# zwang86/FlexFlow

Measured on AMD Instinct MI355X. Metric: samples/sec under auto-searched strategy at 1/2/4/8 MI355X; speedup vs DP, higher is better.
Workload: dtype bf16; 1 GPU; model=bert-large, global_batch=32, seq_len=512, parallelism=single, search=data_parallel, optimizer=adam, params=366426938, hidden=1024, layers=24, heads=16, vocab=30522, vocab_padded=30528

## Files before the change

csrc/kernels/norm.hip:

```cpp
#include "common.h"
#include "ops.h"

namespace ffk {

template <typename T, int NCH>
__global__ void __launch_bounds__(256) ln_fwd_kernel(const T* __restrict__ x, const T* __restrict__ res,
                                                     T* __restrict__ sum_out, const T* __restrict__ gamma,
                                                     const T* __restrict__ beta, T* __restrict__ y,
                                                     float* __restrict__ mean_out, float* __restrict__ rstd_out,
                                                     int rows, int cols, float eps) {
  constexpr int V = 16 / sizeof(T);
  const int lane = threadIdx.x & 63;
  const int wave = (blockIdx.x * blockDim.x + threadIdx.x) >> 6;
  const int nwaves = (gridDim.x * blockDim.x) >> 6;
  for (int row = wave; row < rows; row += nwaves) {
    const int64_t base = (int64_t)row * cols;
    float v[NCH][V];
    float s = 0.f;
#pragma unroll
    for (int c = 0; c < NCH; ++c) {
      const int col = (c * 64 + lane) * V;
      if (col < cols) {
        load16(x + base + col, v[c]);
        if (res) {
          float r[V];
          load16(res + base + col, r);
#pragma unroll
          for (int j = 0; j < V; ++j) v[c][j] += r[j];
          if (sum_out) store16(sum_out + base + col, v[c]);
        }
#pragma unroll
        for (int j = 0; j < V; ++j) s += v[c][j];
      } else {
#pragma unroll
        for (int j = 0; j < V; ++j) v[c][j] = 0.f;
      }
    }
    const float mean = wave_sum(s) / cols;
    float q = 0.f;
#pragma unroll
    for (int c = 0; c < NCH; ++c) {
      const int col = (c * 64 + lane) * V;
      if (col < cols) {
#pragma unroll
        for (int j = 0; j < V; ++j) { const float d = v[c][j] - mean; q += d * d; }
      }
    }
    const float rstd = rsqrtf(wave_sum(q) / cols + eps);
    if (lane == 0) { mean_out[row] = mean; rstd_out[row] = rstd; }
#pragma unroll
    for (int c = 0; c < NCH; ++c) {
      const int col = (c * 64 + lane) * V;
      if (col < cols) {
        float g[V], bb[V], o[V];
        if (gamma) load16(gamma + col, g); else for (int j = 0; j < V; ++j) g[j] = 1.f;
        if (beta) load16(beta + col, bb); else for (int j = 0; j < V; ++j) bb[j] = 0.f;
#pragma unroll
        for (int j = 0; j < V; ++j) o[j] = (v[c][j] - mean) * rstd * g[j] + bb[j];
        store16(y + base + col, o);
      }
    }
  }
}

template <typename T>
__global__ void ln_fwd_generic(const T* __restrict__ x, const T* __restrict__ res, T* __restrict__ sum_out,
                               const T* __restrict__ gamma, const T* __restrict__ beta, T* __restrict__ y,
                               float* __restrict__ mean_out, float* __restrict__ rstd_out, int rows, int cols,
                               float eps) {
  const int lane = threadIdx.x & 63;
  const int wave = (blockIdx.x * blockDim.x + threadIdx.x) >> 6;
  const int nwaves = (gridDim.x * blockDim.x) >> 6;
  for (int row = wave; row < rows; row += nwaves) {
    const int64_t base = (int64_t)row * cols;
    float s = 0.f;
    for (int c = lane; c < cols; c += 64) {
      float v = Cvt<T>::to_f(x[base + c]);
      if (res) { v += Cvt<T>::to_f(res[base + c]); if (sum_out) sum_out[base + c] = Cvt<T>::from_f(v); }
      s += v;
    }
    const float mean = wave_sum(s) / cols;
    float q = 0.f;
    for (int c = lane; c < cols; c += 64) {
      float v = Cvt<T>::to_f(x[base + c]) + (res ? Cvt<T>::to_f(res[base + c]) : 0.f);
      q += (v - mean) * (v - mean);
    }
    const float rstd = rsqrtf(wave_sum(q) / cols + eps);
    if (lane == 0) { mean_out[row] = mean; rstd_out[row] = rstd; }
    for (int c = lane; c < cols; c += 64) {
      float v = Cvt<T>::to_f(x[base + c]) + (res ? Cvt<T>::to_f(res[base + c]) : 0.f);
      float g = gamma ? Cvt<T>::to_f(gamma[c]) : 1.f;
      float b = beta ? Cvt<T>::to_f(beta[c]) : 0.f;
      y[base + c] = Cvt<T>::from_f((v - mean) * rstd * g + b);
    }
  }
}

template <typename T, int NCH, int NT = 256>
__global__ void __launch_bounds__(NT) ln_bwd_kernel(const T* __restrict__ dy, const T* __restrict__ x,
                                                     const T* __restrict__ gamma, const float* __restrict__ mean_in,
                                                     const float* __restrict__ rstd_in, T* __restrict__ dx,
                                                     const T* __restrict__ dres_in, float* __restrict__ pgam,
                                                     float* __restrict__ pbet, float* __restrict__ pdx, int rows,
                                                     int cols, int accumulate) {
  constexpr int V = 16 / sizeof(T);
  const int lane = threadIdx.x & 63;
  const int wave = (blockIdx.x * blockDim.x + threadIdx.x) >> 6;
  const int nwaves = (gridDim.x * blockDim.x) >> 6;
  float pg[NCH][V], pb[NCH][V], pd[NCH][V];
#pragma unroll
  for (int c = 0; c < NCH; ++c)
#pragma unroll
    for (int j = 0; j < V; ++j) { pg[c][j] = 0.f; pb[c][j] = 0.f; pd[c][j] = 0.f; }
  for (int row = wave; row < rows; row += nwaves) {
    const int64_t base = (int64_t)row * cols;
    const float mean = mean_in[row], rstd = rstd_in[row];
    float xh[NCH][V], gy[NCH][V];
    float s1 = 0.f, s2 = 0.f;
#pragma unroll
    for (int c = 0; c < NCH; ++c) {
      const int col = (c * 64 + lane) * V;
      if (col < cols) {
        float xv[V], dv[V], g[V];
        load16(x + base + col, xv);
        load16(dy + base + col, dv);
        if (gamma) load16(gamma + col, g); else for (int j = 0; j < V; ++j) g[j] = 1.f;
#pragma unroll
        for (int j = 0; j < V; ++j) {
          xh[c][j] = (xv[j] - mean) * rstd;
          pg[c][j] += dv[j] * xh[c][j];
          pb[c][j] += dv[j];
          gy[c][j] = dv[j] * g[j];
          s1 += gy[c][j];
          s2 += gy[c][j] * xh[c][j];
        }
      } else {
#pragma unroll
        for (int j = 0; j < V; ++j) { xh[c][j] = 0.f; gy[c][j] = 0.f; }
      }
    }
    s1 = wave_sum(s1) / cols;
    s2 = wave_sum(s2) / cols;
#pragma unroll
    for (int c = 0; c < NCH; ++c) {
      const int col = (c * 64 + lane) * V;
      if (col < cols) {
        float o[V];
#pragma unroll
        for (int j = 0; j < V; ++j) o[j] = rstd * (gy[c][j] - s1 - xh[c][j] * s2);
        if (dres_in) {
          float r[V];
          load16(dres_in + base + col, r);
#pragma unroll
          for (int j = 0; j < V; ++j) o[j] += r[j];
        }
        if (accumulate) {
          float r[V];
          load16(dx + base + col, r);
#pragma unroll
          for (int j = 0; j < V; ++j) o[j] += r[j];
        }
#pragma unroll
        for (int j = 0; j < V; ++j) pd[c][j] += o[j];
        store16(dx + base + col, o);
      }
    }
  }
  extern __shared__ float lds_red[];
  constexpr int NWB = NT / 64;
  const int w = threadIdx.x >> 6;
#pragma unroll
  for (int pass = 0; pass < 3; ++pass) {
    float* slab = pass == 2 ? pdx : (pass ? pbet : pgam);
    if (!slab) continue;
#pragma unroll
    for (int c = 0; c < NCH; ++c) {
      const int col = (c * 64 + lane) * V;
      if (col < cols)
#pragma unroll
        for (int j = 0; j < V; ++j) lds_red[w * cols + col + j] = pass == 2 ? pd[c][j] : (pass ? pb[c][j] : pg[c][j]);
    }
    __syncthreads();
    for (int k = threadIdx.x; k < cols; k += NT) {
      float t = 0.f;
#pragma unroll
      for (int q = 0; q < NWB; ++q) t += lds_red[q * cols + k];
      slab[(int64_t)blockIdx.x * cols + k] = t;
    }
    __syncthreads();
  }
}

template <typename T>
__global__ void ln_bwd_generic(const T* __restrict__ dy, const T* __restrict__ x, const T* __restrict__ gamma,
                               const float* __restrict__ mean_in, const float* __restrict__ rstd_in,
                               T* __restrict__ dx, const T* __restrict__ dres_in, float* __restrict__ dgamma,
                               float* __restrict__ dbeta, int rows, int cols, int accumulate) {
  const int lane = threadIdx.x & 63;
  const int wave = (blockIdx.x * blockDim.x + threadIdx.x) >> 6;
  const int nwaves = (gridDim.x * blockDim.x) >> 6;
  for (int row = wave; row < rows; row += nwaves) {
    const int64_t base = (int64_t)row * cols;
    const float mean = mean_in[row], rstd = rstd_in[row];
    float s1 = 0.f, s2 = 0.f;
    for (int c = lane; c < cols; c += 64) {
      const float xh = (Cvt<T>::to_f(x[base + c]) - mean) * rstd;
      const float d = Cvt<T>::to_f(dy[base + c]);
      const float g = (gamma ? Cvt<T>::to_f(gamma[c]) : 1.f) * d;
      s1 += g; s2 += g * xh;
      if (dgamma) atomicAdd(dgamma + c, d * xh);
      if (dbeta) atomicAdd(dbeta + c, d);
    }
    s1 = wave_sum(s1) / cols;
    s2 = wave_sum(s2) / cols;
    for (int c = lane; c < cols; c += 64) {
      const float xh = (Cvt<T>::to_f(x[base + c]) - mean) * rstd;
      const float g = (gamma ? Cvt<T>::to_f(gamma[c]) : 1.f) * Cvt<T>::to_f(dy[base + c]);
      float o = rstd * (g - s1 - xh * s2);
      if (dres_in) o += Cvt<T>::to_f(dres_in[base + c]);
      if (accumulate) o += Cvt<T>::to_f(dx[base + c]);
      dx[base + c] = Cvt<T>::from_f(o);
    }
  }
}

static bool a16(const void* p) { return ((uintptr_t)p & 15) == 0; }

static bool ln_bwd_wide_on() {
  static int v = -1;
  if (v < 0) {
    const char* e = getenv("FF_LN_BWD_WIDE");
    v = e ? atoi(e) : 0;
  }
  return v != 0;
}

void layernorm_fwd(int dt, const void* x, const void* res, void* sum_out, const void* gamma, const void* beta,
                   void* y, float* mean, float* rstd, int rows, int cols, float eps, hipStream_t st) {
  if (rows == 0) return;
  const int esz = dt == DT_BF16 ? 2 : 4;
  const int V = 16 / esz;
  const bool vec = (cols % V == 0) && a16(x) && a16(y) && (!res || a16(res)) && (!sum_out || a16(sum_out)) &&
                   (!gamma || a16(gamma)) && (!beta || a16(beta));
  const int nch = (cols + 64 * V - 1) / (64 * V);
  const int blocks = std::max(1, std::min((rows + 3) / 4, 4096));
#define LNF(T, N) hipLaunchKernelGGL((ln_fwd_kernel<T, N>), dim3(blocks), dim3(256), 0, st, (const T*)x, (const T*)res, \
                                     (T*)sum_out, (const T*)gamma, (const T*)beta, (T*)y, mean, rstd, rows, cols, eps)
  if (dt == DT_BF16) {
    using T = bf16_t;
    if (vec && nch <= 1) LNF(T, 1); else if (vec && nch <= 2) LNF(T, 2); else if (vec && nch <= 4) LNF(T, 4);
    else if (vec && nch <= 8) LNF(T, 8);
    else hipLaunchKernelGGL(ln_fwd_generic<T>, dim3(blocks), dim3(256), 0, st, (const T*)x, (const T*)res, (T*)sum_out,
                            (const T*)gamma, (const T*)beta, (T*)y, mean, rstd, rows, cols, eps);
  } else {
    using T = float;
    if (vec && nch <= 1) LNF(T, 1); else if (vec && nch <= 2) LNF(T, 2); else if (vec && nch <= 4) LNF(T, 4);
    else if (vec && nch <= 8) LNF(T, 8);
    else hipLaunchKernelGGL(ln_fwd_generic<T>, dim3(blocks), dim3(256), 0, st, (const T*)x, (const T*)res, (T*)sum_out,
                            (const T*)gamma, (const T*)beta, (T*)y, mean, rstd, rows, cols, eps);
  }
#undef LNF
}

int layernorm_bwd_waves(int rows) { return std::max(1, std::min((rows + 15) / 16, 1024)); }
static bool ln_bwd_wide(int cols) { return cols <= 1024 && ln_bwd_wide_on(); }
static int ln_bwd_blocks(int rows, int cols) {
  return ln_bwd_wide(cols) ? std::max(1, std::min((rows + 63) / 64, 256)) : layernorm_bwd_waves(rows);
}

void layernorm_bwd(int dt, const void* dy, const void* x, const void* gamma, const float* mean, const float* rstd,
                   void* dx, const void* dres_in, float* dgamma, float* dbeta, float* dsum, float* ws, int rows,
                   int cols, int accumulate, hipStream_t st, int stage) {
  if (rows == 0) return;
  const int esz = dt == DT_BF16 ? 2 : 4;
  const int V = 16 / esz;
  const bool vec = (cols % V == 0) && a16(x) && a16(dy) && a16(dx) && (!dres_in || a16(dres_in)) &&
                   (!gamma || a16(gamma));
  const int nch = (cols + 64 * V - 1) / (64 * V);
  const bool wide = ln_bwd_wide(cols);
  const int blocks = ln_bwd_blocks(rows, cols);
  const int nw = blocks;
  float* pg = dgamma ? ws : nullptr;
  float* pb = dbeta ? ws + (int64_t)nw * cols : nullptr;
  float* pd = dsum ? ws + 2 * (int64_t)nw * cols : nullptr;
  bool used_slab = false;
  const bool fused_ok = vec && nch <= 4;
  if (stage == 2) {
    if (fused_ok) col_reduce_add3(ws, dgamma, dbeta, dsum, nw, cols, st);
    else if (dsum) bias_act_bwd(dt, dx, nullptr, nullptr, dsum, ws + 2 * (int64_t)nw * cols, rows, cols, ACT_NONE, st, 2);
    return;
  }
#define LNB(T, N) do { used_slab = true; \
    if (wide) hipLaunchKernelGGL((ln_bwd_kernel<T, N, 1024>), dim3(blocks), dim3(1024), 16 * cols * sizeof(float), st, (const T*)dy, \
                                 (const T*)x, (const T*)gamma, mean, rstd, (T*)dx, (const T*)dres_in, pg, pb, pd, rows, cols, accumulate); \
    else hipLaunchKernelGGL((ln_bwd_kernel<T, N>), dim3(blocks), dim3(256), 4 * cols * sizeof(float), st, (const T*)dy, (const T*)x, \
                            (const T*)gamma, mean, rstd, (T*)dx, (const T*)dres_in, pg, pb, pd, rows, cols, accumulate); } while (0)
  if (dt == DT_BF16) {
    using T = bf16_t;
    if (vec && nch <= 1) LNB(T, 1); else if (vec && nch <= 2) LNB(T, 2); else if (vec && nch <= 4) LNB(T, 4);
    else hipLaunchKernelGGL(ln_bwd_generic<T>, dim3(blocks), dim3(256), 0, st, (const T*)dy, (const T*)x,
                            (const T*)gamma, mean, rstd, (T*)dx, (const T*)dres_in, dgamma, dbeta, rows, cols, accumulate);
  } else {
    using T = float;
    if (vec && nch <= 1) LNB(T, 1); else if (vec && nch <= 2) LNB(T, 2); else if (vec && nch <= 4) LNB(T, 4);
    else hipLaunchKernelGGL(ln_bwd_generic<T>, dim3(blocks), dim3(256), 0, st, (const T*)dy, (const T*)x,
                            (const T*)gamma, mean, rstd, (T*)dx, (const T*)dres_in, dgamma, dbeta, rows, cols, accumulate);
  }
#undef LNB
  if (used_slab) {
    if (stage == 0) col_reduce_add3(ws, dgamma, dbeta, dsum, nw, cols, st);
  } else if (dsum) {
    bias_act_bwd(dt, dx, nullptr, nullptr, dsum, ws + 2 * (int64_t)nw * cols, rows, cols, ACT_NONE, st, stage);
  }
  (void)fused_ok;
}

__device__ __forceinline__ float block_sum256(float v, float* sh) {
#pragma unroll
  for (int o = 32; o > 0; o >>= 1) v += __shfl_xor(v, o, 64);
  const int lane = threadIdx.x & 63, wave = threadIdx.x >> 6;
  __syncthreads();
  if (lane == 0) sh[wave] = v;
  __syncthreads();
  return sh[0] + sh[1] + sh[2] + sh[3];
}

template <typename T, int MAXC>
__global__ void __launch_bounds__(256) rms_fwd_kernel(const T* __restrict__ x, const T* __restrict__ w,
                                                      T* __restrict__ y, float* __restrict__ rstd, int rows, int d,
                                                      float eps) {
  __shared__ float sh[4];
  const int tid = threadIdx.x;
  for (int row = blockIdx.x; row < rows; row += gridDim.x) {
    const T* xr = x + (int64_t)row * d;
    float v[MAXC];
    float ss = 0.f;
#pragma unroll
    for (int i = 0; i < MAXC; ++i) {
      const int c = tid + 256 * i;
      v[i] = c < d ? Cvt<T>::to_f(xr[c]) : 0.f;
      ss += v[i] * v[i];
    }
    const float r = rsqrtf(block_sum256(ss, sh) / (float)d + eps);
    if (tid == 0 && rstd) rstd[row] = r;
    T* yr = y + (int64_t)row * d;
#pragma unroll
    for (int i = 0; i < MAXC; ++i) {
      const int c = tid + 256 * i;
      if (c < d) yr[c] = Cvt<T>::from_f(v[i] * r * Cvt<T>::to_f(w[c]));
    }
  }
}

template <typename T, int MAXC>
__global__ void __launch_bounds__(256) rms_bwd_kernel(const T* __restrict__ x, const T* __restrict__ w,
                                                      const T* __restrict__ dy, const float* __restrict__ rstd,
                                                      T* __restrict__ dx, float* __restrict__ dw, int rows, int d) {
  __shared__ float sh[4];
  const int tid = threadIdx.x;
  float dwp[MAXC];
#pragma unroll
  for (int i = 0; i < MAXC; ++i) dwp[i] = 0.f;
  for (int row = blockIdx.x; row < rows; row += gridDim.x) {
    const T* xr = x + (int64_t)row * d;
    const T* dyr = dy + (int64_t)row * d;
    const float r = rstd[row];
    float xv[MAXC], g[MAXC];
    float s = 0.f;
#pragma unroll
    for (int i = 0; i < MAXC; ++i) {
      const int c = tid + 256 * i;
      const float dv = c < d ? Cvt<T>::to_f(dyr[c]) : 0.f;
      xv[i] = c < d ? Cvt<T>::to_f(xr[c]) : 0.f;
      g[i] = c < d ? dv * Cvt<T>::to_f(w[c]) : 0.f;
      s += g[i] * xv[i];
      dwp[i] += dv * xv[i] * r;
    }
    const float k = r * r * r * block_sum256(s, sh) / (float)d;
    T* dxr = dx + (int64_t)row * d;
#pragma unroll
    for (int i = 0; i < MAXC; ++i) {
      const int c = tid + 256 * i;
      if (c < d) dxr[c] = Cvt<T>::from_f(r * g[i] - k * xv[i]);
    }
  }
  if (dw) {
#pragma unroll
    for (int i = 0; i < MAXC; ++i) {
      const int c = tid + 256 * i;
      if (c < d) atomicAdd(dw + c, dwp[i]);
    }
  }
}

void rmsnorm_fwd(int dt, const void* x, const void* w, void* y, float* rstd, int rows, int d, float eps,
                 hipStream_t st) {
  if (rows == 0) return;
  if (dt == DT_BF16) {
    const int g = std::max(1, std::min(rows, 1024));
    if (d <= 256 * 8) hipLaunchKernelGGL((rms_fwd_kernel<bf16_t, 8>), dim3(g), dim3(256), 0, st, (const bf16_t*)x,
                                         (const bf16_t*)w, (bf16_t*)y, rstd, rows, d, eps);
    else hipLaunchKernelGGL((rms_fwd_kernel<bf16_t, 32>), dim3(g), dim3(256), 0, st, (const bf16_t*)x,
                            (const bf16_t*)w, (bf16_t*)y, rstd, rows, d, eps);
  } else {
    const int g = std::max(1, std::min(rows, 1024));
    if (d <= 256 * 8) hipLaunchKernelGGL((rms_fwd_kernel<float, 8>), dim3(g), dim3(256), 0, st, (const float*)x,
                                         (const float*)w, (float*)y, rstd, rows, d, eps);
    else hipLaunchKernelGGL((rms_fwd_kernel<float, 32>), dim3(g), dim3(256), 0, st, (const float*)x,
                            (const float*)w, (float*)y, rstd, rows, d, eps);
  }
}

void rmsnorm_bwd(int dt, const void* x, const void* w, const void* dy, const float* rstd, void* dx, float* dw,
                 int rows, int d, hipStream_t st) {
  if (rows == 0) return;
  const int g = std::max(1, std::min(rows, 1024));
  if (dt == DT_BF16) {
    if (d <= 256 * 8) hipLaunchKernelGGL((rms_bwd_kernel<bf16_t, 8>), dim3(g), dim3(256), 0, st, (const bf16_t*)x,
                                         (const bf16_t*)w, (const bf16_t*)dy, rstd, (bf16_t*)dx, dw, rows, d);
    else hipLaunchKernelGGL((rms_bwd_kernel<bf16_t, 32>), dim3(g), dim3(256), 0, st, (const bf16_t*)x,
                            (const bf16_t*)w, (const bf16_t*)dy, rstd, (bf16_t*)dx, dw, rows, d);
  } else {
    if (d <= 256 * 8) hipLaunchKernelGGL((rms_bwd_kernel<float, 8>), dim3(g), dim3(256), 0, st, (const float*)x,
                                         (const float*)w, (const float*)dy, rstd, (float*)dx, dw, rows, d);
    else hipLaunchKernelGGL((rms_bwd_kernel<float, 32>), dim3(g), dim3(256), 0, st, (const float*)x,
                            (const float*)w, (const float*)dy, rstd, (float*)dx, dw, rows, d);
  }
}

}
```

Measured before the change: 767.1 samples/s.

## Software-prefetch next row in LayerNorm backward using buffer loads and register-held gamma

Adds a new LayerNorm backward kernel that keeps gamma in registers, loads x and dy through raw buffer loads, and prefetches the next row's inputs while the current row's reductions and stores run. The wave reduction now uses ds_swizzle, and a compile-time flag skips the residual and accumulate loads when neither is present. The old kernel is kept as a non-prefetching variant for some shapes, and the env-gated 1024-thread wide variant is removed. The aim is to hide global memory latency in a bandwidth-bound kernel, at the cost of higher register pressure and hand-tuned FMA ordering meant to match the old numerics.

New measurement: 769.8 samples/s, median of 6. Within noise of the previous version (+0.4%).

```diff
diff --git a/csrc/kernels/norm.hip b/csrc/kernels/norm.hip
--- a/csrc/kernels/norm.hip
+++ b/csrc/kernels/norm.hip
@@ -96,8 +96,38 @@
   }
 }
 
-template <typename T, int NCH, int NT = 256>
-__global__ void __launch_bounds__(NT) ln_bwd_kernel(const T* __restrict__ dy, const T* __restrict__ x,
+template <int NCH, int V>
+__device__ __forceinline__ void ln_bwd_fold(const float (&pg)[NCH][V], const float (&pb)[NCH][V],
+                                            const float (&pd)[NCH][V], float* __restrict__ pgam,
+                                            float* __restrict__ pbet, float* __restrict__ pdx, int cols) {
+  extern __shared__ float lds_red[];
+  constexpr int NT = 256, NWB = NT / 64;
+  const int lane = threadIdx.x & 63;
+  const int w = threadIdx.x >> 6;
+#pragma unroll
+  for (int pass = 0; pass < 3; ++pass) {
+    float* slab = pass == 2 ? pdx : (pass ? pbet : pgam);
+    if (!slab) continue;
+#pragma unroll
+    for (int c = 0; c < NCH; ++c) {
+      const int col = (c * 64 + lane) * V;
+      if (col < cols)
+#pragma unroll
+        for (int j = 0; j < V; ++j) lds_red[w * cols + col + j] = pass == 2 ? pd[c][j] : (pass ? pb[c][j] : pg[c][j]);
+    }
+    __syncthreads();
+    for (int k = threadIdx.x; k < cols; k += NT) {
+      float t = 0.f;
+#pragma unroll
+      for (int q = 0; q < NWB; ++q) t += lds_red[q * cols + k];
+      slab[(int64_t)blockIdx.x * cols + k] = t;
+    }
+    __syncthreads();
+  }
+}
+
+template <typename T, int NCH>
+__global__ void __launch_bounds__(256) ln_bwd_kernel_nopf(const T* __restrict__ dy, const T* __restrict__ x,
                                                      const T* __restrict__ gamma, const float* __restrict__ mean_in,
                                                      const float* __restrict__ rstd_in, T* __restrict__ dx,
                                                      const T* __restrict__ dres_in, float* __restrict__ pgam,
@@ -166,29 +196,162 @@
       }
     }
   }
-  extern __shared__ float lds_red[];
-  constexpr int NWB = NT / 64;
-  const int w = threadIdx.x >> 6;
-#pragma unroll
-  for (int pass = 0; pass < 3; ++pass) {
-    float* slab = pass == 2 ? pdx : (pass ? pbet : pgam);
-    if (!slab) continue;
-#pragma unroll
-    for (int c = 0; c < NCH; ++c) {
-      const int col = (c * 64 + lane) * V;
-      if (col < cols)
-#pragma unroll
-        for (int j = 0; j < V; ++j) lds_red[w * cols + col + j] = pass == 2 ? pd[c][j] : (pass ? pb[c][j] : pg[c][j]);
-    }
-    __syncthreads();
-    for (int k = threadIdx.x; k < cols; k += NT) {
-      float t = 0.f;
-#pragma unroll
-      for (int q = 0; q < NWB; ++q) t += lds_red[q * cols + k];
-      slab[(int64_t)blockIdx.x * cols + k] = t;
-    }
-    __syncthreads();
-  }
+  ln_bwd_fold<NCH, V>(pg, pb, pd, pgam, pbet, pdx, cols);
+}
+
+typedef uint32_t u32x4 __attribute__((ext_vector_type(4)));
+
+template <typename T>
+__device__ __forceinline__ void unpack16(const u32x4& raw, float* out) {
+  const T* e = reinterpret_cast<const T*>(&raw);
+#pragma unroll
+  for (int i = 0; i < (int)(16 / sizeof(T)); ++i) out[i] = Cvt<T>::to_f(e[i]);
+}
+template <typename T>
+__device__ __forceinline__ u32x4 pack16(const float* in) {
+  u32x4 raw;
+  T* e = reinterpret_cast<T*>(&raw);
+#pragma unroll
+  for (int i = 0; i < (int)(16 / sizeof(T)); ++i) e[i] = Cvt<T>::from_f(in[i]);
+  return raw;
+}
+__device__ __forceinline__ __amdgpu_buffer_rsrc_t row_rsrc(const void* p, int bytes) {
+  return __builtin_amdgcn_make_buffer_rsrc(const_cast<void*>(p), (short)0, bytes, 0x00020000);
+}
+
+template <int O>
+__device__ __forceinline__ float swz_xor(float v) {
+  return __int_as_float(__builtin_amdgcn_ds_swizzle(__float_as_int(v), (O << 10) | 0x1f));
+}
+__device__ __forceinline__ float wave_sum_swz(float v) {
+  v += __shfl_xor(v, 32, 64);
+  v += swz_xor<16>(v);
+  v += swz_xor<8>(v);
+  v += swz_xor<4>(v);
+  v += swz_xor<2>(v);
+  v += swz_xor<1>(v);
+  return v;
+}
+
+template <typename T, int NCH, bool EXTRA>
+__global__ void __launch_bounds__(256) ln_bwd_kernel(const T* __restrict__ dy, const T* __restrict__ x,
+                                                     const T* __restrict__ gamma, const float* __restrict__ mean_in,
+                                                     const float* __restrict__ rstd_in, T* __restrict__ dx,
+                                                     const T* __restrict__ dres_in, float* __restrict__ pgam,
+                                                     float* __restrict__ pbet, float* __restrict__ pdx, int rows,
+                                                     int cols, int accumulate) {
+  constexpr int V = 16 / sizeof(T);
+  const int lane = threadIdx.x & 63;
+  const int wave = __builtin_amdgcn_readfirstlane((blockIdx.x * blockDim.x + threadIdx.x) >> 6);
+  const int nwaves = (gridDim.x * blockDim.x) >> 6;
+  const int row_bytes = cols * (int)sizeof(T);
+  float pg[NCH][V], pb[NCH][V], pd[NCH][V];
+  u32x4 gr[NCH];
+#pragma unroll
+  for (int c = 0; c < NCH; ++c) {
+    float one[V];
+#pragma unroll
+    for (int j = 0; j < V; ++j) { pg[c][j] = 0.f; pb[c][j] = 0.f; pd[c][j] = 0.f; one[j] = 1.f; }
+    const int col = (c * 64 + lane) * V;
+    gr[c] = (gamma && col < cols) ? *reinterpret_cast<const u32x4*>(gamma + col) : pack16<T>(one);
+  }
+  u32x4 rx[NCH], rd[NCH], rr[EXTRA ? NCH : 1], ra[EXTRA ? NCH : 1];
+  float rmean = 0.f, rrstd = 0.f;
+  auto fetch = [&](int r) {
+    const int64_t base = (int64_t)r * cols;
+    const __amdgpu_buffer_rsrc_t sx = row_rsrc(x + base, row_bytes), sd = row_rsrc(dy + base, row_bytes);
+#pragma unroll
+    for (int c = 0; c < NCH; ++c) {
+      const int off = (c * 64 + lane) * 16;
+      rx[c] = __builtin_amdgcn_raw_buffer_load_b128(sx, off, 0, 0);
+      rd[c] = __builtin_amdgcn_raw_buffer_load_b128(sd, off, 0, 0);
+    }
+    rmean = mean_in[r];
+    rrstd = rstd_in[r];
+  };
+  auto fetch_extra = [&](int r) {
+    const int64_t base = (int64_t)r * cols;
+    if (dres_in) {
+      const __amdgpu_buffer_rsrc_t sr = row_rsrc(dres_in + base, row_bytes);
+#pragma unroll
+      for (int c = 0; c < (EXTRA ? NCH : 0); ++c) rr[c] = __builtin_amdgcn_raw_buffer_load_b128(sr, (c * 64 + lane) * 16, 0, 0);
+    }
+    if (accumulate) {
+      const __amdgpu_buffer_rsrc_t sa = row_rsrc(dx + base, row_bytes);
+#pragma unroll
+      for (int c = 0; c < (EXTRA ? NCH : 0); ++c) ra[c] = __builtin_amdgcn_raw_buffer_load_b128(sa, (c * 64 + lane) * 16, 0, 0);
+    }
+  };
+  auto do_row = [&](int row) {
+#pragma clang fp contract(off)
+    const int64_t base = (int64_t)row * cols;
+    const float mean = rmean, rstd = rrstd;
+    float xh[NCH][V], gy[NCH][V];
+    float s1 = 0.f, s2 = 0.f;
+#pragma unroll
+    for (int c = 0; c < NCH; ++c) {
+      asm volatile("" : "+v"(gr[c]));
+      const int col = (c * 64 + lane) * V;
+      if (col < cols) {
+        float xv[V], dv[V], g[V];
+        unpack16<T>(rx[c], xv);
+        unpack16<T>(rd[c], dv);
+        unpack16<T>(gr[c], g);
+#pragma unroll
+        for (int j = 0; j < V; ++j) {
+          const bool uneven = sizeof(T) == 2 && c == 1;
+          xh[c][j] = (xv[j] - mean) * rstd;
+          pg[c][j] = __builtin_fmaf(dv[j], xh[c][j], pg[c][j]);
+          pb[c][j] += dv[j];
+          gy[c][j] = dv[j] * g[j];
+          s1 = uneven && (j == 0 || j == 2) ? __builtin_fmaf(dv[j], g[j], s1) : s1 + gy[c][j];
+          s2 = uneven && j < 3 ? __builtin_fmaf(gy[c][j], xh[c][j], s2) : s2 + gy[c][j] * xh[c][j];
+          asm volatile("" : "+v"(s2));
+        }
+      }
+    }
+    const int nrow = row + nwaves;
+    if (nrow < rows) fetch(nrow);
+    s1 = wave_sum_swz(s1) / cols;
+    s2 = wave_sum_swz(s2) / cols;
+    const __amdgpu_buffer_rsrc_t so = row_rsrc(dx + base, row_bytes);
+#pragma unroll
+    for (int c = 0; c < NCH; ++c) {
+      const int col = (c * 64 + lane) * V;
+      u32x4 po = {};
+      if (col < cols) {
+        float o[V];
+#pragma unroll
+        for (int j = 0; j < V; ++j)
+          o[j] = rstd * (c == NCH - 1 && j >= V - 2 ? gy[c][j] - s1 - xh[c][j] * s2
+                                                    : __builtin_fmaf(-xh[c][j], s2, gy[c][j] - s1));
+        if (EXTRA && dres_in) {
+          float r[V];
+          unpack16<T>(rr[c], r);
+#pragma unroll
+          for (int j = 0; j < V; ++j) o[j] += r[j];
+        }
+        if (EXTRA && accumulate) {
+          float r[V];
+          unpack16<T>(ra[c], r);
+#pragma unroll
+          for (int j = 0; j < V; ++j) o[j] += r[j];
+        }
+#pragma unroll
+        for (int j = 0; j < V; ++j) pd[c][j] += o[j];
+        po = pack16<T>(o);
+      }
+      __builtin_amdgcn_raw_buffer_store_b128(po, so, col * (int)sizeof(T), 0, 0);
+    }
+    if (EXTRA && nrow < rows) fetch_extra(nrow);
+  };
+  if (wave < rows) {
+    fetch(wave);
+    fetch_extra(wave);
+    do_row(wave);
+    for (int row = wave + nwaves; row < rows; row += nwaves) do_row(row);
+  }
+  ln_bwd_fold<NCH, V>(pg, pb, pd, pgam, pbet, pdx, cols);
 }
 
 template <typename T>
@@ -225,15 +388,6 @@
 }
 
 static bool a16(const void* p) { return ((uintptr_t)p & 15) == 0; }
-
-static bool ln_bwd_wide_on() {
-  static int v = -1;
-  if (v < 0) {
-    const char* e = getenv("FF_LN_BWD_WIDE");
-    v = e ? atoi(e) : 0;
-  }
-  return v != 0;
-}
 
 void layernorm_fwd(int dt, const void* x, const void* res, void* sum_out, const void* gamma, const void* beta,
                    void* y, float* mean, float* rstd, int rows, int cols, float eps, hipStream_t st) {
@@ -263,10 +417,6 @@
 }
 
 int layernorm_bwd_waves(int rows) { return std::max(1, std::min((rows + 15) / 16, 1024)); }
-static bool ln_bwd_wide(int cols) { return cols <= 1024 && ln_bwd_wide_on(); }
-static int ln_bwd_blocks(int rows, int cols) {
-  return ln_bwd_wide(cols) ? std::max(1, std::min((rows + 63) / 64, 256)) : layernorm_bwd_waves(rows);
-}
 
 void layernorm_bwd(int dt, const void* dy, const void* x, const void* gamma, const float* mean, const float* rstd,
                    void* dx, const void* dres_in, float* dgamma, float* dbeta, float* dsum, float* ws, int rows,
@@ -277,8 +427,7 @@
   const bool vec = (cols % V == 0) && a16(x) && a16(dy) && a16(dx) && (!dres_in || a16(dres_in)) &&
                    (!gamma || a16(gamma));
   const int nch = (cols + 64 * V - 1) / (64 * V);
-  const bool wide = ln_bwd_wide(cols);
-  const int blocks = ln_bwd_blocks(rows, cols);
+  const int blocks = layernorm_bwd_waves(rows);
   const int nw = blocks;
   float* pg = dgamma ? ws : nullptr;
   float* pb = dbeta ? ws + (int64_t)nw * cols : nullptr;
@@ -290,23 +439,28 @@
     else if (dsum) bias_act_bwd(dt, dx, nullptr, nullptr, dsum, ws + 2 * (int64_t)nw * cols, rows, cols, ACT_NONE, st, 2);
     return;
   }
-#define LNB(T, N) do { used_slab = true; \
-    if (wide) hipLaunchKernelGGL((ln_bwd_kernel<T, N, 1024>), dim3(blocks), dim3(1024), 16 * cols * sizeof(float), st, (const T*)dy, \
-                                 (const T*)x, (const T*)gamma, mean, rstd, (T*)dx, (const T*)dres_in, pg, pb, pd, rows, cols, accumulate); \
-    else hipLaunchKernelGGL((ln_bwd_kernel<T, N>), dim3(blocks), dim3(256), 4 * cols * sizeof(float), st, (const T*)dy, (const T*)x, \
-                            (const T*)gamma, mean, rstd, (T*)dx, (const T*)dres_in, pg, pb, pd, rows, cols, accumulate); } while (0)
+#define LNB2(T, N, E) do { used_slab = true; \
+    hipLaunchKernelGGL((ln_bwd_kernel<T, N, E>), dim3(blocks), dim3(256), 4 * cols * sizeof(float), st, (const T*)dy, (const T*)x, \
+                       (const T*)gamma, mean, rstd, (T*)dx, (const T*)dres_in, pg, pb, pd, rows, cols, accumulate); } while (0)
+#define LNB1(T, N) do { used_slab = true; \
+    hipLaunchKernelGGL((ln_bwd_kernel_nopf<T, N>), dim3(blocks), dim3(256), 4 * cols * sizeof(float), st, (const T*)dy, (const T*)x, \
+                       (const T*)gamma, mean, rstd, (T*)dx, (const T*)dres_in, pg, pb, pd, rows, cols, accumulate); } while (0)
+#define LNB(T, N) do { if (!(dres_in || accumulate)) LNB2(T, N, false); \
+                       else if constexpr (sizeof(T) == 2 && N == 2) LNB1(T, N); else LNB2(T, N, true); } while (0)
   if (dt == DT_BF16) {
     using T = bf16_t;
-    if (vec && nch <= 1) LNB(T, 1); else if (vec && nch <= 2) LNB(T, 2); else if (vec && nch <= 4) LNB(T, 4);
+    if (vec && nch <= 1) LNB(T, 1); else if (vec && nch <= 2) LNB(T, 2); else if (vec && nch <= 4) LNB1(T, 4);
     else hipLaunchKernelGGL(ln_bwd_generic<T>, dim3(blocks), dim3(256), 0, st, (const T*)dy, (const T*)x,
                             (const T*)gamma, mean, rstd, (T*)dx, (const T*)dres_in, dgamma, dbeta, rows, cols, accumulate);
   } else {
     using T = float;
-    if (vec && nch <= 1) LNB(T, 1); else if (vec && nch <= 2) LNB(T, 2); else if (vec && nch <= 4) LNB(T, 4);
+    if (vec && nch <= 1) LNB(T, 1); else if (vec && nch <= 2) LNB(T, 2); else if (vec && nch <= 4) LNB1(T, 4);
     else hipLaunchKernelGGL(ln_bwd_generic<T>, dim3(blocks), dim3(256), 0, st, (const T*)dy, (const T*)x,
                             (const T*)gamma, mean, rstd, (T*)dx, (const T*)dres_in, dgamma, dbeta, rows, cols, accumulate);
   }
 #undef LNB
+#undef LNB2
+#undef LNB1
   if (used_slab) {
     if (stage == 0) col_reduce_add3(ws, dgamma, dbeta, dsum, nw, cols, st);
   } else if (dsum) {
```
